# thunlp/ConvDR

Hardware: AMD Instinct MI355X
Metric: passages encoded/sec + query x passage IP-scored/sec, 768-d (higher is better)
Workload: dtype bf16

## Files before the change

convdr_amd/csrc/encoder_kernels.hpp:

```cpp
#pragma once
#include "../../include/convdr_hip.h"
#include "dropout.hpp"
#include "gemm_nt.hpp"

namespace convdr {

static __global__ void __launch_bounds__(256) k_seq_pack(const void* __restrict__ ids_v, int ids32,
                                                  const int64_t* __restrict__ mask, const int32_t* __restrict__ lens,
                                                  int B, int L, const int32_t* __restrict__ cu, int kind, int pad_idx,
                                                  int max_pos, int vocab, int32_t* __restrict__ tok_id,
                                                  int32_t* __restrict__ tok_pos, int32_t* __restrict__ status) {
  const int lane = threadIdx.x & 63;
  const int b = blockIdx.x * 4 + (threadIdx.x >> 6);
  if (b >= B) return;
  const int base = cu[b], end = cu[b + 1];
  const int64_t* ids = (const int64_t*)ids_v;
  const int32_t* ids_i = (const int32_t*)ids_v;
  const int len_b = lens[b];
  int kept = 0, nonpad = 0;
  int flags = 0;
  for (int l0 = 0; l0 < L; l0 += 64) {
    const int l = l0 + lane;
    const bool valid = l < L;
    int64_t id = valid ? (ids32 ? (int64_t)ids_i[(int64_t)b * L + l] : ids[(int64_t)b * L + l]) : (int64_t)pad_idx;
// ... 166 lines not shown
    const int e0 = 256 * j + 4 * lane;
    uint2 o;
    o.x = pack_bf16x2((x[j].x - mean) * rstd * gg[j].x + bb[j].x, (x[j].y - mean) * rstd * gg[j].y + bb[j].y);
    o.y = pack_bf16x2((x[j].z - mean) * rstd * gg[j].z + bb[j].z, (x[j].w - mean) * rstd * gg[j].w + bb[j].w);
    *(uint2*)(Xb + row * H + e0) = o;
  }
}

template <int J>
static __global__ void __launch_bounds__(256) k_slab_finish_ln(const float* __restrict__ slab, int nsplit, int64_t rows,
                                                               const float* __restrict__ bias, const bf16_t* __restrict__ R,
                                                               const float* __restrict__ g, const float* __restrict__ b, float eps,
                                                               bf16_t* __restrict__ Xb) {
  constexpr int H = 256 * J;
  const int lane = threadIdx.x & 63;
  const int64_t row = (int64_t)blockIdx.x * 4 + (threadIdx.x >> 6);
  if (row >= rows) return;
  float4 x[J], gg[J], bb[J], part[4][J];
  uint2 r[J];
#pragma unroll
  for (int j = 0; j < J; ++j) {
    const int e0 = 256 * j + 4 * lane;
    x[j] = *(const float4*)(bias + e0);
    gg[j] = *(const float4*)(g + e0);
    bb[j] = *(const float4*)(b + e0);
    r[j] = *(const uint2*)(R + row * H + e0);
#pragma unroll
    for (int s = 0; s < 4; ++s)
      part[s][j] = *(const float4*)(slab + ((int64_t)(s < nsplit ? s : 0) * rows + row) * H + e0);
  }
  float sum = 0.f;
#pragma unroll
  for (int j = 0; j < J; ++j) {
#pragma unroll
    for (int s = 0; s < 4; ++s)
      if (s < nsplit) { x[j].x += part[s][j].x; x[j].y += part[s][j].y; x[j].z += part[s][j].z; x[j].w += part[s][j].w; }
    x[j].x += __uint_as_float(r[j].x << 16); x[j].y += __uint_as_float(r[j].x & 0xffff0000u);
    x[j].z += __uint_as_float(r[j].y << 16); x[j].w += __uint_as_float(r[j].y & 0xffff0000u);
    sum += x[j].x + x[j].y + x[j].z + x[j].w;
  }
  const float mean = wave_sum(sum) / (float)H;
  float q = 0.f;
#pragma unroll
  for (int j = 0; j < J; ++j) {
    const float a = x[j].x - mean, c = x[j].y - mean, d = x[j].z - mean, e = x[j].w - mean;
    q += a * a + c * c + d * d + e * e;
  }
  const float rstd = rsqrtf(wave_sum(q) / (float)H + eps);
#pragma unroll
  for (int j = 0; j < J; ++j) {
    const int e0 = 256 * j + 4 * lane;
    uint2 o;
    o.x = pack_bf16x2((x[j].x - mean) * rstd * gg[j].x + bb[j].x, (x[j].y - mean) * rstd * gg[j].y + bb[j].y);
    o.y = pack_bf16x2((x[j].z - mean) * rstd * gg[j].z + bb[j].z, (x[j].w - mean) * rstd * gg[j].w + bb[j].w);
    *(uint2*)(Xb + row * H + e0) = o;
  }
}

inline int64_t g_ln_rows = 1;
static inline void launch_layernorm_bf16(const float* Y, int64_t rows, int H, const float* g, const float* b, float eps, bf16_t* Xb,
                                         hipStream_t st) {
  if (g_ln_rows && H == 768)
    hipLaunchKernelGGL(k_layernorm_rows<3>, dim3((unsigned)((rows + 3) / 4)), dim3(256), 0, st, Y, rows, g, b, eps, Xb);
  else
    hipLaunchKernelGGL(k_layernorm, dim3((unsigned)((rows + 3) / 4)), dim3(256), 0, st, Y, rows, H, g, b, eps, Xb, (float*)nullptr);
}

static __global__ void __launch_bounds__(256) k_gather_cls(const int32_t* __restrict__ cu, int B, int H,
                                                    const bf16_t* __restrict__ Xb, const float* __restrict__ Xf,
                                                    bf16_t* __restrict__ Ob, float* __restrict__ Of) {
  const int lane = threadIdx.x & 63;
  const int b = blockIdx.x * 4 + (threadIdx.x >> 6);
  if (b >= B) return;
  const int64_t row = cu[b];
  for (int e0 = 4 * lane; e0 < H; e0 += 256) {
    if (Ob) *(uint2*)(Ob + (int64_t)b * H + e0) = *(const uint2*)(Xb + row * H + e0);
    if (Of) *(float4*)(Of + (int64_t)b * H + e0) = *(const float4*)(Xf + row * H + e0);
  }
}

static __global__ void __launch_bounds__(256) k_masked_mean(const bf16_t* __restrict__ X, const int32_t* __restrict__ cu,
                                                     const int32_t* __restrict__ lens, int H, bf16_t* __restrict__ Ob,
                                                     float* __restrict__ Of) {
  const int b = blockIdx.x, c = 4 * threadIdx.x;
  if (c >= H) return;
  const int64_t base = cu[b];
  const int len = lens[b];
  float4 s = make_float4(0.f, 0.f, 0.f, 0.f);
  for (int t = 0; t < len; ++t) {
    const uint2 v = *(const uint2*)(X + (base + t) * H + c);
    s.x += __uint_as_float(v.x << 16); s.y += __uint_as_float(v.x & 0xffff0000u);
    s.z += __uint_as_float(v.y << 16); s.w += __uint_as_float(v.y & 0xffff0000u);
  }
  const float inv = 1.f / (float)len;
  s.x *= inv; s.y *= inv; s.z *= inv; s.w *= inv;
  if (Of) *(float4*)(Of + (int64_t)b * H + c) = s;
  if (Ob) {
    uint2 o;
    o.x = pack_bf16x2(s.x, s.y);
    o.y = pack_bf16x2(s.z, s.w);
    *(uint2*)(Ob + (int64_t)b * H + c) = o;
  }
}

enum { EPI_BF16 = 0, EPI_GELU_BF16 = 1, EPI_RESID_F32 = 2, EPI_QKV = 3, EPI_F32 = 4,
       EPI_GELU_SAVE = 5,
       EPI_SLAB_F32 = 7,
       EPI_GELU_BLK = 8,
       EPI_GELU_GP = 9,
       EPI_MUL_GP = 10 };
__host__ __device__ inline int64_t hm_blocked_offset(int64_t t, int f, int N) {
  return ((t >> 5) * (N >> 3) + (f >> 3)) * 256 + (t & 31) * 8 + (f & 7);
}

struct GemmArgs {
  const bf16_t* W;
  const bf16_t* X;
  int64_t rows;
  int N, K;
  int64_t ldw, ldx;
  int k_split_len;
  const float* bias;
  bf16_t* Cb;
  bf16_t* Cb2;
  float* Cf;
  const bf16_t* Gp;
  const bf16_t* R;
  const float* Rf;
  bf16_t *Qo, *Ko, *Vt;
  int third0;
  int qk_blocked;
  int H;
  int64_t ldt;
  int tilesN, tilesT;
  int tile_hint;
  int nt_out;
  int dbg_same_tile;
  int dbg_skip_epi;
  int dbg_prelanded;
  unsigned long long* trace;
  unsigned long long* clock_probe;
  DropSite drop;
};


__device__ __forceinline__ float gelu_tail(float x) {
  const float t = fminf(fabsf(x), 9.f);
  float p = fmaf(t, 0.0041585f, -0.04571999f);
  p = fmaf(p, t, -0.46495319f);
  p = fmaf(p, t, -1.14955714f);
  const float q = __builtin_amdgcn_exp2f(fmaf(p, t, -1.f));
  return fmaf(-t, q, fmaxf(x, 0.f));
}
__device__ __forceinline__ void gelu_tail2(float& x0, float& x1) {
  f32x2_t t, r;
  float a, b;
  const float nine = 9.f;
  asm("v_min_f32 %0, |%1|, %2" : "=v"(a) : "v"(x0), "s"(nine));
  asm("v_min_f32 %0, |%1|, %2" : "=v"(b) : "v"(x1), "s"(nine));
  t.x = a; t.y = b;
  asm("v_max_f32 %0, 0, %1" : "=v"(a) : "v"(x0));
  asm("v_max_f32 %0, 0, %1" : "=v"(b) : "v"(x1));
  r.x = a; r.y = b;
  const f32x2_t c3 = {0.0041585f, 0.0041585f}, c2 = {-0.04571999f, -0.04571999f}, c1 = {-0.46495319f, -0.46495319f},
                c0 = {-1.14955714f, -1.14955714f}, m1 = {-1.f, -1.f};
  f32x2_t p = __builtin_elementwise_fma(t, c3, c2);
  p = __builtin_elementwise_fma(p, t, c1);
  p = __builtin_elementwise_fma(p, t, c0);
  p = __builtin_elementwise_fma(p, t, m1);
  f32x2_t q;
  q.x = __builtin_amdgcn_exp2f(p.x);
  q.y = __builtin_amdgcn_exp2f(p.y);
  r = __builtin_elementwise_fma(-t, q, r);
  x0 = r.x; x1 = r.y;
}

__device__ __forceinline__ float gelu_grad(float x) {
  const float t = fminf(fabsf(x), 9.f);
  float p = fmaf(t, 0.0041585f, -0.04571999f);
  p = fmaf(p, t, -0.46495319f);
  p = fmaf(p, t, -1.14955714f);
  const float q = __builtin_amdgcn_exp2f(fmaf(p, t, -1.f));
  const float cdf = x >= 0.f ? 1.f - q : q;
  const float e = __builtin_amdgcn_exp2f(-0.7213475204444817f * x * x);
  return fmaf(x * 0.3989422804014327f, e, cdf);
}

__device__ __forceinline__ void gelu_tail2_gp(float& x0, float& x1, float& g0, float& g1) {
  f32x2_t t, r;
  float a, b;
  const float nine = 9.f;
  asm("v_min_f32 %0, |%1|, %2" : "=v"(a) : "v"(x0), "s"(nine));
  asm("v_min_f32 %0, |%1|, %2" : "=v"(b) : "v"(x1), "s"(nine));
  t.x = a; t.y = b;
  asm("v_max_f32 %0, 0, %1" : "=v"(a) : "v"(x0));
  asm("v_max_f32 %0, 0, %1" : "=v"(b) : "v"(x1));
  r.x = a; r.y = b;
  const f32x2_t c3 = {0.0041585f, 0.0041585f}, c2 = {-0.04571999f, -0.04571999f}, c1 = {-0.46495319f, -0.46495319f},
                c0 = {-1.14955714f, -1.14955714f}, m1 = {-1.f, -1.f};
  f32x2_t p = __builtin_elementwise_fma(t, c3, c2);
  p = __builtin_elementwise_fma(p, t, c1);
  p = __builtin_elementwise_fma(p, t, c0);
  p = __builtin_elementwise_fma(p, t, m1);
  f32x2_t q;
  q.x = __builtin_amdgcn_exp2f(p.x);
  q.y = __builtin_amdgcn_exp2f(p.y);
  const f32x2_t d4 = {-0.0117551f, -0.0117551f}, d3 = {0.09555683f, 0.09555683f}, d2 = {0.64461331f, 0.64461331f},
                d1 = {0.79644568f, 0.79644568f}, d0 = {-0.99992798f, -0.99992798f}, half = {0.5f, 0.5f};
  f32x2_t m = __builtin_elementwise_fma(t, d4, d3);
  m = __builtin_elementwise_fma(m, t, d2);
  m = __builtin_elementwise_fma(m, t, d1);
  m = __builtin_elementwise_fma(m, t, d0);
  const f32x2_t hr = __builtin_elementwise_fma(q, m, half);
  g0 = 0.5f + __builtin_copysignf(hr.x, x0);
  g1 = 0.5f + __builtin_copysignf(hr.y, x1);
  r = __builtin_elementwise_fma(-t, q, r);
  x0 = r.x; x1 = r.y;
}

template <class T>
struct CTile {
  static constexpr int PASSES = (T::TL * T::TR * 2) / T::STAGE_BYTES;
  static constexpr int NTP = T::NT / PASSES;
  static constexpr int ROWS = T::TL / PASSES;
  static_assert(PASSES >= 1 && PASSES * NTP == T::NT, "a pass is a whole number of MFMA column blocks");
  static constexpr int HALF = ROWS / 2, HALF_BYTES = HALF * T::TR * 2;
  struct Base { uint32_t lo, hi; };
  __device__ static __forceinline__ Base contiguous(const char* sC) {
    static_assert(2 * HALF_BYTES <= T::STAGE_BYTES, "a parked pass must fit the idle stage");
    return Base{lds_off(sC), lds_off(sC) + HALF_BYTES};
  }
  static constexpr int CW = T::MT * 4;
  static constexpr int RW = NTP * 32;
  static constexpr int W_BYTES = RW * CW * 16;
  static constexpr int W_STORES = RW * CW / 64;
  static_assert(W_BYTES * T::WAVES <= 2 * HALF_BYTES && (64 % CW) == 0, "wave-local park must fit the pass image");
  __device__ static __forceinline__ uint32_t wave_base(Base sC, int wave) {
    constexpr int PER_HALF = HALF_BYTES / W_BYTES;
    return (wave >= PER_HALF ? sC.hi + (wave - PER_HALF) * W_BYTES : sC.lo + wave * W_BYTES);
  }
  __device__ static __forceinline__ void put_w(uint32_t wb, const WavePos<T>& w, int mt, int ntl, int g, uint2 o) {
    const int row = ntl * 32 + w.li;
    lds_write_b64_hidden(wb + row * (CW * 16) + (((mt * 4 + g) ^ (row & (CW - 1))) << 4) + w.hi * 8, (u32x2_t){o.x, o.y});
  }
  template <int C0, int CN>
  __device__ static __forceinline__ void store_w_part(bool nt, uint32_t wb, int lane, bf16_t* dst, int64_t ld, int64_t row_limit,
                                                      int64_t col_limit) {
    constexpr int RPI = 64 / CN, N_ST = RW / RPI;
    static_assert(64 % CN == 0 && N_ST % 4 == 0, "store_w_part geometry");
    const int r0 = lane / CN, c = C0 + (lane - r0 * CN);
    const int64_t nv = col_limit - c * 8;
#pragma unroll
    for (int i0 = 0; i0 < N_ST; i0 += 4) {
      u32x4_t v[4];
      auto at = [&](int i) {
        const int row = i * RPI + r0;
        return wb + row * (CW * 16) + ((c ^ (row & (CW - 1))) << 4);
      };
      lds_read4_b128_hidden(at(i0), at(i0 + 1), at(i0 + 2), at(i0 + 3), v[0], v[1], v[2], v[3]);
#pragma unroll
      for (int j = 0; j < 4; ++j) {
        const int row = (i0 + j) * RPI + r0;
        bf16_t* pr = dst + (int64_t)row * ld + c * 8;
        if (row < row_limit && nv > 0) {
          if (nv >= 8) {
            if (nt) store16<true>(pr, v[j]);
            else store16<false>(pr, v[j]);
          }
          else *(uint2*)pr = make_uint2(v[j].x, v[j].y);
        }
      }
    }
  }
  __device__ static __forceinline__ void store_w(bool nt, uint32_t wb, int lane, bf16_t* dst, int64_t ld, int64_t row_limit,
                                                 int64_t col_limit) {
    constexpr int RPI = 64 / CW;
    const int r0 = lane / CW, c = lane - r0 * CW;
    const int64_t nv = col_limit - c * 8;
    static_assert(W_STORES % 4 == 0, "lds_read4_b128_hidden reads four chunks");
#pragma unroll
    for (int i0 = 0; i0 < W_STORES; i0 += 4) {
      u32x4_t v[4];
      auto at = [&](int i) {
        const int row = i * RPI + r0;
        return wb + row * (CW * 16) + ((c ^ (row & (CW - 1))) << 4);
      };
      lds_read4_b128_hidden(at(i0), at(i0 + 1), at(i0 + 2), at(i0 + 3), v[0], v[1], v[2], v[3]);
#pragma unroll
      for (int j = 0; j < 4; ++j) {
        const int row = (i0 + j) * RPI + r0;
        bf16_t* pr = dst + (int64_t)row * ld + c * 8;
        if (row < row_limit && nv > 0) {
          if (nv >= 8) {
            if (nt) store16<true>(pr, v[j]);
            else store16<false>(pr, v[j]);
          }
          else *(uint2*)pr = make_uint2(v[j].x, v[j].y);
        }
      }
    }
  }
};

template <int EPI, class T>
static __global__ void __launch_bounds__(T::THREADS, 2) k_gemm(const GemmArgs a) {
  extern __shared__ __attribute__((aligned(16))) char smem[];
  using CT = CTile<T>;
  const WavePos<T> w;
  const int64_t ldw = a.ldw ? a.ldw : a.K, ldx = a.ldx ? a.ldx : a.K;
  int kbeg = 0, klen = a.K;
  if constexpr (EPI == EPI_SLAB_F32) {
    if (a.k_split_len) { kbeg = blockIdx.y * a.k_split_len; klen = a.k_split_len; }
  }
  const uint32_t ntiles = (uint32_t)a.tilesN * a.tilesT;
  const uint32_t xcd = blockIdx.x & 7u, q8 = ntiles >> 3, r8 = ntiles & 7u;
  const uint32_t chunk_base = xcd < r8 ? xcd * (q8 + 1) : r8 * (q8 + 1) + (xcd - r8) * q8;
  const uint32_t chunk_len = q8 + (xcd < r8 ? 1u : 0u);
  const uint32_t stride = (gridDim.x + 7u) >> 3;
  uint32_t idx = blockIdx.x >> 3;
  if (idx >= chunk_len) return;
  if (a.clock_probe && blockIdx.x == 0 && blockIdx.y == 0 && threadIdx.x == 0) {
    a.clock_probe[0] = __builtin_amdgcn_s_memtime();
    a.clock_probe[1] = __builtin_amdgcn_s_memrealtime();
  }

  struct Coord { int64_t t0; int n0; int swap; };
  auto decode = [&](uint32_t i) {
    const uint32_t logical = chunk_base + i;
    int tt = logical / a.tilesN, tn = logical - tt * a.tilesN;
    if (a.dbg_same_tile) { tt = 0; tn = 0; }
    Coord c;
    c.t0 = (int64_t)tt * T::TL;
    c.n0 = tn * T::TR;
    c.swap = false;
    if constexpr (EPI == EPI_QKV) c.swap = c.n0 + a.third0 * a.H >= 2 * a.H;
    return c;
  };
  auto tile_src = [&](const Coord& c) {
    return c.swap ? TileSrc<T>(a.X, ldx, a.rows, a.W, ldw, a.N, c.t0, c.n0, w)
                  : TileSrc<T>(a.W + kbeg, ldw, a.N, a.X + kbeg, ldx, a.rows, c.n0, c.t0, w);
  };

  constexpr bool R3 = T::WAVES == 8;
  R3Slots st{0, 0};
  auto sbias_of = [&](R3Slots s) { return (float*)(smem + (s.rs == 2 ? 0 : s.rs + 1) * T::R_BYTES); };
  auto tile_src_all = [&](const Coord& cc) {
    return cc.swap ? TileSrcAll<T>(a.X, ldx, a.rows, a.W, ldw, a.N, cc.t0, cc.n0, w)
                   : TileSrcAll<T>(a.W + kbeg, ldw, a.N, a.X + kbeg, ldx, a.rows, cc.n0, cc.t0, w);
  };
  float* sbias = R3 ? sbias_of(st) : (float*)(smem + T::SMEM_BYTES);
  int trace_tile = 0;
#ifdef CONVDR_ENABLE_TRACE
#define CONVDR_TRACE(ph)                                                                                       \
  if (a.trace && threadIdx.x == 0 && trace_tile < 64)                                                          \
    a.trace[((size_t)blockIdx.x * 64 + trace_tile) * 16 + (ph)] = __builtin_amdgcn_s_memtime();
#else
#define CONVDR_TRACE(ph)
#endif
  auto bias_slice = [&](const Coord& cc) {
    const int f = cc.n0 + (int)threadIdx.x;
    return (!cc.swap && a.bias && threadIdx.x < T::TR && f < a.N) ? a.bias[f] : 0.f;
  };
  Coord c = decode(idx);
  int buf = 0;
  bool landed = false;
  if (threadIdx.x < T::TR) sbias[threadIdx.x] = bias_slice(c);
  TileSrc<T> src = tile_src(c);
  TileSrcAll<T> src3 = tile_src_all(c);
  if constexpr (R3) gemm_r3_prologue<T>(src3, a.K, smem, w, st, false);
  else gemm_issue_stage<T>(src, 0, smem + buf * T::STAGE_BYTES, w);
  __syncthreads();
  for (;;) {
    const uint32_t next = idx + stride;
    const bool has_next = next < chunk_len;
    const Coord cn = has_next ? decode(next) : c;
    GemmAcc<T> acc;
    float bias_lane[T::NT];
    if (c.swap) {
      acc.zero();
#pragma unroll
      for (int nt = 0; nt < T::NT; ++nt) {
        const int f = c.n0 + w.l_index(nt);
        bias_lane[nt] = a.bias[f < a.N ? f : a.N - 1];
      }
    } else {
#pragma unroll
      for (int nt = 0; nt < T::NT; ++nt) bias_lane[nt] = 0.f;
#pragma unroll
      for (int mt = 0; mt < T::MT; ++mt) {
        u32x4_t bq[4];
        const uint32_t sb = lds_off(sbias);
        lds_read4_b128_hidden(sb + w.r_base(mt, 0) * 4, sb + w.r_base(mt, 1) * 4, sb + w.r_base(mt, 2) * 4,
                              sb + w.r_base(mt, 3) * 4, bq[0], bq[1], bq[2], bq[3]);
#pragma unroll
        for (int g = 0; g < 4; ++g)
#pragma unroll
          for (int nt = 0; nt < T::NT; ++nt) {
            acc.c[mt][nt][4 * g + 0] = __uint_as_float(bq[g].x); acc.c[mt][nt][4 * g + 1] = __uint_as_float(bq[g].y);
            acc.c[mt][nt][4 * g + 2] = __uint_as_float(bq[g].z); acc.c[mt][nt][4 * g + 3] = __uint_as_float(bq[g].w);
          }
      }
    }
    float bias_next = has_next ? bias_slice(cn) : 0.f;
    constexpr bool RES_PRE = EPI == EPI_RESID_F32 && T::WAVES == 4;
    uint2 res_pre[RES_PRE ? T::NT : 1][T::MT][4];
    if constexpr (RES_PRE) {
      if (a.Rf == nullptr) {
#pragma unroll
        for (int nt = 0; nt < T::NT; ++nt) {
          const int64_t t = c.t0 + w.l_index(nt);
          const int64_t tc = t < a.rows ? t : a.rows - 1;
#pragma unroll
          for (int mt = 0; mt < T::MT; ++mt)
#pragma unroll
            for (int g = 0; g < 4; ++g) {
              int f = c.n0 + w.r_base(mt, g);
              f = f < a.N ? f : a.N - 4;
              res_pre[nt][mt][g] = *(const uint2*)(a.R + tc * a.N + f);
            }
        }
      }
    }
    CONVDR_TRACE(0)
    int idle;
    if constexpr (R3) {
      st = gemm_nt_mainloop_r3<T>(src3, c.swap ? a.K : klen, smem, acc, w, st, true, true, landed || a.dbg_prelanded,
                                  (a.trace && trace_tile == 8) ? a.trace + ((size_t)blockIdx.x * 64 + 56) * 16 : nullptr);
      idle = 0;
      sbias = sbias_of(st);
    } else {
    idle = gemm_nt_mainloop<T>(src, c.swap ? a.K : klen, smem, acc, w, buf, true, landed,
                               (a.trace && trace_tile == 8) ? a.trace + ((size_t)blockIdx.x * 64 + 56) * 16 : nullptr);
    }
    landed = false;
    constexpr bool GP_PRE = EPI == EPI_MUL_GP;
    u32x4_t gp_pre[GP_PRE ? T::NT : 1][GP_PRE ? T::MT : 1][2];
    if constexpr (GP_PRE) {
      int tid_p = threadIdx.x;
      asm volatile("" : "+v"(tid_p));
      const WavePos<T> wp(tid_p);
      const int64_t rows32p = (a.rows + 31) & ~(int64_t)31;
#pragma unroll
      for (int nt = 0; nt < T::NT; ++nt) {
        const int64_t tb = c.t0 + (wp.wl * T::NT + nt) * 32;
        const int64_t tbc = tb < rows32p ? tb : 0;
#pragma unroll
        for (int mt = 0; mt < T::MT; ++mt) {
          const int f0 = c.n0 + wp.wr * T::MT * 32 + mt * 32;
          const int f0c = f0 < a.N ? f0 : 0;
          const bf16_t* blk = a.Gp + ((tbc >> 5) * (a.N >> 3) + (f0c >> 3)) * 256 + wp.li * 8;
#pragma unroll
          for (int j = 0; j < 2; ++j)
            gp_pre[nt][mt][j] = __builtin_nontemporal_load((const u32x4_t*)(blk + (int64_t)(2 * j + wp.hi) * 256));
        }
      }
    }
    asm volatile("" : "+v"(bias_next));
    if constexpr (RES_PRE) {
#pragma unroll
      for (int nt = 0; nt < T::NT; ++nt)
#pragma unroll
        for (int mt = 0; mt < T::MT; ++mt)
#pragma unroll
          for (int g = 0; g < 4; ++g) asm volatile("" : "+v"(res_pre[nt][mt][g].x), "+v"(res_pre[nt][mt][g].y));
    }
#pragma unroll
    for (int i = 0; i < T::NT; ++i) asm volatile("" : "+v"(bias_lane[i]));
    if (threadIdx.x < T::TR) sbias[threadIdx.x] = bias_next;
    CONVDR_TRACE(1)
    if (has_next) {
      if constexpr (R3) {
        src3 = tile_src_all(cn);
        gemm_r3_prologue<T>(src3, a.K, smem, w, st, false);
      } else {
        src = tile_src(cn);
        gemm_issue_stage<T>(src, 0, smem + idle * T::STAGE_BYTES, w);
      }
    }
    typename CT::Base sC;
    if constexpr (R3) {
      static_assert(T::R_BYTES >= CT::HALF_BYTES && 3 * T::R_BYTES + 2 * T::L_BYTES + (T::L_BYTES >= CT::HALF_BYTES ? 0 : CT::HALF_BYTES) <= 160 * 1024,
                    "parked pass: one dead R slot + one dead L slot (or the spare LDS behind the slots)");
      sC = typename CT::Base{lds_off(smem + (st.rs == 0 ? 2 : st.rs - 1) * T::R_BYTES),
                             T::L_BYTES >= CT::HALF_BYTES ? lds_off(smem + 3 * T::R_BYTES + (st.ls ^ 1) * T::L_BYTES)
                                                          : lds_off(smem + 3 * T::R_BYTES + 2 * T::L_BYTES)};
    } else {
      sC = CT::contiguous(smem + (idle ^ 1) * T::STAGE_BYTES);
    }
    int tid_e = threadIdx.x;
    asm volatile("" : "+v"(tid_e));
    const WavePos<T> we(tid_e);
    const int64_t t0 = c.t0;
    const int n0 = c.n0;

    if (a.dbg_skip_epi == 1) {
      float s = 0.f;
#pragma unroll
      for (int mt = 0; mt < T::MT; ++mt)
#pragma unroll
        for (int nt = 0; nt < T::NT; ++nt)
#pragma unroll
          for (int r = 0; r < 16; ++r) s += acc.c[mt][nt][r];
      if (s == 12345.678f) a.Cb[0] = f32_to_bf16(s);
    } else if (c.swap) {
      lds_barrier();
#pragma unroll
      for (int pass = 0; pass < CT::PASSES; ++pass) {
        const uint32_t wb = CT::wave_base(sC, we.wave);
#pragma unroll
        for (int ntl = 0; ntl < CT::NTP; ++ntl) {
          const int nt = pass * CT::NTP + ntl;
          const float bv = bias_lane[nt];
#pragma unroll
          for (int mt = 0; mt < T::MT; ++mt)
#pragma unroll
            for (int g = 0; g < 4; ++g) {
              const f32x16& v = acc.c[mt][nt];
              uint2 o;
              o.x = pack_bf16x2(v[4 * g + 0] + bv, v[4 * g + 1] + bv);
              o.y = pack_bf16x2(v[4 * g + 2] + bv, v[4 * g + 3] + bv);
              CT::put_w(wb, we, mt, ntl, g, o);
            }
        }
        if (pass == CT::PASSES - 1 && has_next) {
          lds_dma_wait_all();
          landed = true;
        }
        const int row0 = (we.wl * T::NT + pass * CT::NTP) * 32, col0 = we.wr * T::MT * 32;
        CT::store_w(a.nt_out != 0, wb, we.lane, a.Vt + (int64_t)(n0 + (a.third0 - 2) * a.H + row0) * a.ldt + t0 + col0, a.ldt,
                    a.N - n0 - row0, a.rows - t0 - col0);
      }
    } else if (EPI == EPI_GELU_BLK || (EPI == EPI_QKV && a.qk_blocked)) {
      lds_barrier();
      CONVDR_TRACE(2)
      const int64_t rows32 = (a.rows + 31) & ~(int64_t)31;
      bf16_t* dstm = a.Cb;
      int oct_w = a.N >> 3, f0 = n0;
      if constexpr (EPI == EPI_QKV) {
        const int na = n0 + a.third0 * a.H;
        dstm = na < a.H ? a.Qo : a.Ko;
        f0 = na < a.H ? na : na - a.H;
        oct_w = a.H >> 3;
      }
#pragma unroll
      for (int nt = 0; nt < T::NT; ++nt) {
        const int64_t tb = t0 + (we.wl * T::NT + nt) * 32;
        if (nt == T::NT - 1 && has_next) {
          lds_dma_wait_all();
          landed = true;
        }
        bf16_t* blk = dstm + ((tb >> 5) * oct_w + ((f0 + we.wr * T::MT * 32) >> 3)) * 256 + we.li * 8;
#pragma unroll
        for (int mt = 0; mt < T::MT; ++mt)
#pragma unroll
          for (int j = 0; j < 2; ++j) {
            uint2 o[2];
#pragma unroll
            for (int e = 0; e < 2; ++e) {
              const int g = 2 * j + e;
              const f32x16& v = acc.c[mt][nt];
              float y0 = v[4 * g + 0], y1 = v[4 * g + 1], y2 = v[4 * g + 2], y3 = v[4 * g + 3];
              if constexpr (EPI == EPI_GELU_BLK) { gelu_tail2(y0, y1); gelu_tail2(y2, y3); }
              o[e].x = pack_bf16x2(y0, y1);
              o[e].y = pack_bf16x2(y2, y3);
            }
            const auto sx = __builtin_amdgcn_permlane32_swap(o[0].x, o[1].x, false, false);
            const auto sy = __builtin_amdgcn_permlane32_swap(o[0].y, o[1].y, false, false);
            u32x4_t q;
            q.x = sx[0]; q.y = sy[0]; q.z = sx[1]; q.w = sy[1];
            if (tb < rows32 && n0 + we.wr * T::MT * 32 + mt * 32 < a.N)
              store16<NT_GEMM_BLK>(blk + (int64_t)(mt * 4 + 2 * j + we.hi) * 256, q);
          }
      }
      CONVDR_TRACE(6)
    } else {
      lds_barrier();
      CONVDR_TRACE(2)
      const bool full_n = n0 + T::TR <= a.N;
      constexpr bool BF16_OUT = EPI == EPI_BF16 || EPI == EPI_GELU_BF16 || EPI == EPI_QKV || EPI == EPI_GELU_SAVE ||
                                EPI == EPI_GELU_GP || EPI == EPI_MUL_GP;
      constexpr bool GP = EPI == EPI_GELU_GP || EPI == EPI_MUL_GP;
      const int64_t rows32 = (a.rows + 31) & ~(int64_t)31;
      constexpr int NOUT = EPI == EPI_GELU_SAVE ? 2 : 1;
#pragma unroll
      for (int out = 0; out < NOUT; ++out)
#pragma unroll
        for (int pass = 0; pass < CT::PASSES; ++pass) {
          const uint32_t wb = CT::wave_base(sC, we.wave);
          constexpr bool HALVES = BF16_OUT && T::MT >= 4 && CT::NTP == 1;
          bf16_t* wdst = nullptr;
          int64_t wld = 0, wrows = 0, wcols = 0;
          if constexpr (HALVES) {
            bf16_t* dst;
            int64_t cols;
            if constexpr (EPI == EPI_QKV) {
              const int na = n0 + a.third0 * a.H;
              dst = na < a.H ? a.Qo + t0 * a.H + na : a.Ko + t0 * a.H + (na - a.H);
              wld = a.H; cols = T::TR;
            } else {
              dst = (out ? a.Cb2 : a.Cb) + t0 * a.N + n0;
              wld = a.N; cols = a.N - n0;
            }
            const int row0 = (we.wl * T::NT + pass * CT::NTP) * 32, col0 = we.wr * T::MT * 32;
            wdst = dst + (int64_t)row0 * wld + col0; wrows = a.rows - t0 - row0; wcols = cols - col0;
          }
#pragma unroll
          for (int ntl = 0; ntl < CT::NTP; ++ntl) {
            const int nt = pass * CT::NTP + ntl;
            const int64_t t = t0 + we.l_index(nt);
            const bool t_ok = t < a.rows;
            const int64_t tc = t_ok ? t : a.rows - 1;
            uint2 res[T::MT][4];
            u32x4_t gpq[GP ? T::MT : 1][2];
            bf16_t* gp_blk = nullptr;
            bool gp_ok = false;
            if constexpr (GP) {
              const int64_t tb = t0 + (we.wl * T::NT + nt) * 32;
              bf16_t* img = EPI == EPI_GELU_GP ? a.Cb2 : const_cast<bf16_t*>(a.Gp);
              gp_blk = img + ((tb >> 5) * (a.N >> 3) + ((n0 + we.wr * T::MT * 32) >> 3)) * 256 + we.li * 8;
              gp_ok = tb < rows32;
              if constexpr (EPI == EPI_MUL_GP) {
#pragma unroll
                for (int mt = 0; mt < T::MT; ++mt)
#pragma unroll
                  for (int j = 0; j < 2; ++j) gpq[mt][j] = gp_pre[nt][mt][j];
              }
            }
            if constexpr (EPI == EPI_RESID_F32) {
              if (a.Rf == nullptr) {
#pragma unroll
                for (int mt = 0; mt < T::MT; ++mt)
#pragma unroll
                  for (int g = 0; g < 4; ++g) {
                    if constexpr (RES_PRE) {
                      res[mt][g] = res_pre[nt][mt][g];
                    } else {
                      int f = n0 + we.r_base(mt, g);
                      f = (full_n || f < a.N) ? f : a.N - 4;
                      res[mt][g] = *(const uint2*)(a.R + tc * a.N + f);
                    }
                  }
              }
            }
            uint2 gpq_o0 = make_uint2(0u, 0u), gpq_o1 = make_uint2(0u, 0u);
#pragma unroll
            for (int mt = 0; mt < T::MT; ++mt)
#pragma unroll
              for (int g = 0; g < 4; ++g) {
                const int fl = we.r_base(mt, g);
                const int f = n0 + fl;
                const f32x16& v = acc.c[mt][nt];
                float y0 = v[4 * g + 0], y1 = v[4 * g + 1], y2 = v[4 * g + 2], y3 = v[4 * g + 3];
                if constexpr (EPI == EPI_GELU_BF16 || EPI == EPI_GELU_SAVE) {
                  if (out == 0) {
                    gelu_tail2(y0, y1); gelu_tail2(y2, y3);
                  }
                }
                if constexpr (EPI == EPI_GELU_GP) {
                  float d0, d1, d2, d3;
                  gelu_tail2_gp(y0, y1, d0, d1); gelu_tail2_gp(y2, y3, d2, d3);
                  uint2& dq = (g & 1) ? gpq_o1 : gpq_o0;
                  dq.x = pack_bf16x2(d0, d1);
                  dq.y = pack_bf16x2(d2, d3);
                  if (g & 1) {
                    const auto sx = __builtin_amdgcn_permlane32_swap(gpq_o0.x, gpq_o1.x, false, false);
                    const auto sy = __builtin_amdgcn_permlane32_swap(gpq_o0.y, gpq_o1.y, false, false);
                    u32x4_t q4;
                    q4.x = sx[0]; q4.y = sy[0]; q4.z = sx[1]; q4.w = sy[1];
                    if (gp_ok && (full_n || f < a.N))
                      store16<true>(gp_blk + (int64_t)(mt * 4 + (g & 2) + we.hi) * 256, q4);
                  }
                }
                if constexpr (EPI == EPI_MUL_GP) {
                  if (!(g & 1)) {
                    const u32x4_t q4 = gpq[mt][g >> 1];
                    const auto sx = __builtin_amdgcn_permlane32_swap(q4.x, q4.z, false, false);
                    const auto sy = __builtin_amdgcn_permlane32_swap(q4.y, q4.w, false, false);
                    gpq_o0 = make_uint2(sx[0], sy[0]);
                    gpq_o1 = make_uint2(sx[1], sy[1]);
                  }
                  const uint2 dq = (g & 1) ? gpq_o1 : gpq_o0;
                  y0 *= __uint_as_float(dq.x << 16); y1 *= __uint_as_float(dq.x & 0xffff0000u);
                  y2 *= __uint_as_float(dq.y << 16); y3 *= __uint_as_float(dq.y & 0xffff0000u);
                }
                if constexpr (EPI == EPI_RESID_F32) {
                  if (a.drop.thresh) {
                    float m0, m1, m2, m3;
                    drop_hidden4(a.drop, t, f, a.N, m0, m1, m2, m3);
                    y0 *= m0; y1 *= m1; y2 *= m2; y3 *= m3;
                  }
                  if (a.Rf) {
                    const int fc = (full_n || f < a.N) ? f : a.N - 4;
                    const float4 r = *(const float4*)(a.Rf + tc * a.N + fc);
                    y0 += r.x; y1 += r.y; y2 += r.z; y3 += r.w;
                  } else {
                    const uint2 r = res[mt][g];
                    y0 += __uint_as_float(r.x << 16); y1 += __uint_as_float(r.x & 0xffff0000u);
                    y2 += __uint_as_float(r.y << 16); y3 += __uint_as_float(r.y & 0xffff0000u);
                  }
                }
                if constexpr (BF16_OUT) {
                  uint2 o;
                  o.x = pack_bf16x2(y0, y1);
                  o.y = pack_bf16x2(y2, y3);
                  CT::put_w(wb, we, mt, ntl, g, o);
                  if constexpr (HALVES) {
                    if (mt == T::MT / 2 - 1 && g == 3) {
                      if (out == NOUT - 1 && pass == CT::PASSES - 1 && has_next) { lds_dma_wait_all(); landed = true; }
                      CT::template store_w_part<0, CT::CW / 2>(a.nt_out != 0, wb, we.lane, wdst, wld, wrows, wcols);
                    }
                  }
                } else if (t_ok && (full_n || f < a.N)) {
                  if constexpr (EPI == EPI_SLAB_F32) {
                    *(float4*)(a.Cf + ((int64_t)blockIdx.y * a.rows + t) * a.N + f) = make_float4(y0, y1, y2, y3);
                  } else {
                    *(float4*)(a.Cf + t * a.N + f) = make_float4(y0, y1, y2, y3);
                  }
                }
              }
          }
          CONVDR_TRACE(3 + 4 * pass)
          if constexpr (BF16_OUT) {
            CONVDR_TRACE(4 + 4 * pass)
            if (out == NOUT - 1 && pass == CT::PASSES - 1 && has_next) {
              lds_dma_wait_all();
              landed = true;
            }
            CONVDR_TRACE(5 + 4 * pass)
            if (a.dbg_skip_epi != 3) {
              bf16_t* dst;
              int64_t ldo, cols;
              if constexpr (EPI == EPI_QKV) {
                const int na = n0 + a.third0 * a.H;
                dst = na < a.H ? a.Qo + t0 * a.H + na : a.Ko + t0 * a.H + (na - a.H);
// ... 268 lines not shown
```

convdr_amd/csrc/gemm_nt.hpp:

```cpp
#pragma once
#include "common.hpp"

namespace convdr {

constexpr int GEMM_BK = 64;

typedef const __attribute__((address_space(1))) void* gptr_t;
typedef __attribute__((address_space(3))) void* lptr_t;

__device__ __forceinline__ void glds16(const void* g, void* lds_wave_base) {
  __builtin_amdgcn_global_load_lds((gptr_t)g, (lptr_t)lds_wave_base, 16, 0, 0);
}
template <bool NT, class V>
__device__ __forceinline__ void store16(void* p, const V& v) {
  static_assert(sizeof(V) == 16, "16-byte store");
  typedef uint32_t raw4_t __attribute__((ext_vector_type(4)));
  if constexpr (NT) __builtin_nontemporal_store(__builtin_bit_cast(raw4_t, v), (raw4_t*)p);
  else *(V*)p = v;
}
constexpr bool NT_GEMM_BLK = true;
constexpr bool NT_CTILE = true;
constexpr bool NT_ATT = true;
constexpr bool NT_LN = true;
template <int AUX>
__device__ __forceinline__ void glds16_aux(const void* g, void* lds_wave_base) {
  __builtin_amdgcn_global_load_lds((gptr_t)g, (lptr_t)lds_wave_base, 16, 0, AUX);
}

__device__ __forceinline__ void lds_dma_wait_all() { asm volatile("s_waitcnt vmcnt(0)" ::: "memory"); }

__device__ __forceinline__ void lds_barrier() { asm volatile("s_waitcnt lgkmcnt(0)\n\ts_barrier" ::: "memory"); }

typedef uint32_t u32x4_t __attribute__((ext_vector_type(4)));
typedef uint32_t u32x2_t __attribute__((ext_vector_type(2)));
__device__ __forceinline__ uint32_t lds_off(const void* p) {
  return (uint32_t)(uintptr_t)(__attribute__((address_space(3))) const char*)p;
}
__device__ __forceinline__ void lds_write_b64_hidden(uint32_t addr, u32x2_t v) {
  asm volatile("ds_write_b64 %0, %1" ::"v"(addr), "v"(v) : "memory");
}
__device__ __forceinline__ void lds_read4_b128_hidden(uint32_t a0, uint32_t a1, uint32_t a2, uint32_t a3, u32x4_t& v0,
                                                      u32x4_t& v1, u32x4_t& v2, u32x4_t& v3) {
  asm volatile(
      "ds_read_b128 %0, %4\n\tds_read_b128 %1, %5\n\tds_read_b128 %2, %6\n\tds_read_b128 %3, %7\n\t"
      "s_waitcnt lgkmcnt(0)"
      : "=&v"(v0), "=&v"(v1), "=&v"(v2), "=&v"(v3)
      : "v"(a0), "v"(a1), "v"(a2), "v"(a3)
      : "memory");
}

typedef _Float16 f16x8 __attribute__((ext_vector_type(8)));
template <bool F16>
__device__ __forceinline__ f32x16 mfma_32x32x16(const bf16x8& a, const bf16x8& b, const f32x16& c) {
  if constexpr (F16)
    return __builtin_amdgcn_mfma_f32_32x32x16_f16(__builtin_bit_cast(f16x8, a), __builtin_bit_cast(f16x8, b), c, 0, 0, 0);
  else
    return __builtin_amdgcn_mfma_f32_32x32x16_bf16(a, b, c, 0, 0, 0);
}

template <int WR_, int WL_, int MT_, int NT_>
struct TileCfg {
  static constexpr int WR = WR_, WL = WL_, MT = MT_, NT = NT_;
  static constexpr int TR = WR * MT * 32, TL = WL * NT * 32;
  static constexpr int WAVES = WR * WL, THREADS = WAVES * 64;
  static constexpr int DMA_WAVES = WAVES == 8 ? 4 : WAVES;
  static constexpr int DMA_FIRST = WAVES - DMA_WAVES;
  static constexpr int R_BYTES = TR * 128, L_BYTES = TL * 128;
  static constexpr int STAGE_BYTES = R_BYTES + L_BYTES;
  static constexpr int SMEM_BYTES = 2 * STAGE_BYTES;
  static constexpr int MIN_WAVES_PER_SIMD = THREADS >= 512 ? 2 : 2;
};
using Tile128 = TileCfg<2, 2, 2, 2>;
using Tile256 = TileCfg<2, 4, 4, 2>;
using TileTall = TileCfg<2, 4, 4, 1>;
using TileWide = TileCfg<4, 2, 2, 2>;

template <class T>
struct GemmAcc {
  f32x16 c[T::MT][T::NT];
  __device__ __forceinline__ void zero() {
#pragma unroll
    for (int i = 0; i < T::MT; ++i)
#pragma unroll
      for (int j = 0; j < T::NT; ++j)
#pragma unroll
        for (int r = 0; r < 16; ++r) c[i][j][r] = 0.f;
  }
};

template <class T>
struct WavePos {
  int lane, wave, wr, wl, hi, li;
  __device__ __forceinline__ WavePos() : WavePos((int)threadIdx.x) {}
  __device__ __forceinline__ explicit WavePos(int tid) {
    lane = tid & 63;
    wave = __builtin_amdgcn_readfirstlane(tid >> 6);
    wr = wave / T::WL;
    wl = wave - wr * T::WL;
    hi = lane >> 5;
    li = lane & 31;
  }
  __device__ __forceinline__ int r_base(int mt, int g) const { return (wr * T::MT + mt) * 32 + 8 * g + 4 * hi; }
  __device__ __forceinline__ int r_index(int mt, int r) const { return (wr * T::MT + mt) * 32 + (r & 3) + 8 * (r >> 2) + 4 * hi; }
  __device__ __forceinline__ int l_index(int nt) const { return (wl * T::NT + nt) * 32 + li; }
};

typedef int32_t i32x4_t __attribute__((ext_vector_type(4)));

struct StageSrc {
  __amdgpu_buffer_rsrc_t rsrc;
  uint32_t voff;
  uint32_t round_pitch;
};

template <int WAVES, int FIRST>
__device__ __forceinline__ StageSrc gemm_stage_src(const bf16_t* __restrict__ G, int64_t ld, int64_t row0, int64_t nrows,
                                                    int wave, int lane) {
  wave = wave >= FIRST ? wave - FIRST : 0;
  StageSrc s;
  int64_t bytes = (nrows - row0) * ld * 2;
  bytes = bytes < 0 ? 0 : (bytes > 0xffffffffll ? 0xffffffffll : bytes);
  const uint64_t base = (uint64_t)(G + row0 * ld);
  const uint32_t lo = __builtin_amdgcn_readfirstlane((uint32_t)base);
  const uint32_t hi = __builtin_amdgcn_readfirstlane((uint32_t)(base >> 32));
  const uint32_t nb = __builtin_amdgcn_readfirstlane((uint32_t)bytes);
  s.rsrc = __builtin_amdgcn_make_buffer_rsrc((void*)(((uint64_t)hi << 32) | lo), 0, nb, 0x00020000);
  const int row = wave * 8 + (lane >> 3);
  const int gch = (lane & 7) ^ ((row >> 1) & 7);
  s.voff = (uint32_t)(row * ld * 2) + gch * 16;
  s.round_pitch = __builtin_amdgcn_readfirstlane((uint32_t)(8 * WAVES * ld * 2));
  return s;
}

template <int ROWS, int WAVES, int FIRST, int AUX = 0>
__device__ __forceinline__ void gemm_stage(const StageSrc& s, int kt, char* lds_tile, int wave) {
  if (FIRST > 0 && wave < FIRST) return;
  wave -= FIRST;
  constexpr int ROUNDS = ROWS / (8 * WAVES);
  static_assert(ROUNDS * 8 * WAVES == ROWS, "tile rows must be a multiple of 8 * waves");
#pragma unroll
  for (int i = 0; i < ROUNDS; ++i)
    __builtin_amdgcn_raw_ptr_buffer_load_lds(s.rsrc, (lptr_t)(lds_tile + (i * WAVES + wave) * 8 * 128), 16, s.voff,
                                             i * s.round_pitch + kt * (GEMM_BK * 2), 0, AUX);
}

template <class T>
struct TileSrc {
  StageSrc R, L;
  __device__ __forceinline__ TileSrc(const bf16_t* __restrict__ Rp, int64_t ldr, int64_t nR, const bf16_t* __restrict__ Lp,
                                     int64_t ldl, int64_t nL, int64_t r0, int64_t l0, const WavePos<T>& w)
      : R(gemm_stage_src<T::DMA_WAVES, T::DMA_FIRST>(Rp, ldr, r0, nR, w.wave, w.lane)),
        L(gemm_stage_src<T::DMA_WAVES, T::DMA_FIRST>(Lp, ldl, l0, nL, w.wave, w.lane)) {}
};

template <class T>
__device__ __forceinline__ void gemm_issue_stage(const TileSrc<T>& src, int kt, char* stage, const WavePos<T>& w) {
  gemm_stage<T::TR, T::DMA_WAVES, T::DMA_FIRST>(src.R, kt, stage, w.wave);
  gemm_stage<T::TL, T::DMA_WAVES, T::DMA_FIRST>(src.L, kt, stage + T::R_BYTES, w.wave);
}

template <class T, bool F16 = false>
__device__ __forceinline__ int gemm_nt_mainloop(const TileSrc<T>& src, int K, char* smem, GemmAcc<T>& acc,
                                                const WavePos<T>& w, int first_buf = 0, bool stage0_in_flight = false,
                                                bool stage0_landed = false, unsigned long long* step_trace = nullptr) {
  const int nk = K / GEMM_BK;
  const int sw = (w.lane >> 1) & 7;
  const int offR = (w.wr * T::MT * 32 + w.li) * 128;
  const int offL = T::R_BYTES + (w.wl * T::NT * 32 + w.li) * 128;

  if (!stage0_in_flight) gemm_issue_stage<T>(src, 0, smem + first_buf * T::STAGE_BYTES, w);

  for (int kt = 0; kt < nk; ++kt) {
    const int buf = (kt + first_buf) & 1;
#ifdef CONVDR_ENABLE_TRACE
#define CONVDR_STEP_TRACE(i) \
  if (step_trace && kt == 6 + (i) / 5 && w.lane == 0) step_trace[w.wave * 8 + (i)] = __builtin_amdgcn_s_memtime();
#else
#define CONVDR_STEP_TRACE(i)
#endif
    CONVDR_STEP_TRACE(5)
    CONVDR_STEP_TRACE(0)
    if (kt > 0 || !stage0_landed) lds_dma_wait_all();
    CONVDR_STEP_TRACE(1)
    lds_barrier();
    CONVDR_STEP_TRACE(2)
    if (kt + 1 < nk) gemm_issue_stage<T>(src, kt + 1, smem + (buf ^ 1) * T::STAGE_BYTES, w);
    CONVDR_STEP_TRACE(3)
    const char* tR = smem + buf * T::STAGE_BYTES + offR;
    const char* tL = smem + buf * T::STAGE_BYTES + offL;
    bf16x8 fa[2][T::MT], fb[2][T::NT];
    auto load_frags = [&](int s, int set) {
      const int ch = ((2 * s + w.hi) ^ sw) * 16;
#pragma unroll
      for (int j = 0; j < T::NT; ++j) fb[set][j] = *(const bf16x8*)(tL + j * 32 * 128 + ch);
#pragma unroll
      for (int i = 0; i < T::MT; ++i) fa[set][i] = *(const bf16x8*)(tR + i * 32 * 128 + ch);
    };
    load_frags(0, 0);
#pragma unroll
    for (int s = 0; s < 4; ++s) {
      if (s + 1 < 4) load_frags(s + 1, (s + 1) & 1);
#pragma unroll
      for (int i = 0; i < T::MT; ++i)
#pragma unroll
        for (int j = 0; j < T::NT; ++j)
          acc.c[i][j] = mfma_32x32x16<F16>(fa[s & 1][i], fb[s & 1][j], acc.c[i][j]);
      if (s + 1 < 4) {
#pragma unroll
        for (int r = 0; r < T::MT + T::NT && r < T::MT * T::NT; ++r) {
          __builtin_amdgcn_sched_group_barrier(0x008, 1, 0);
          __builtin_amdgcn_sched_group_barrier(0x100, 1, 0);
        }
        __builtin_amdgcn_sched_group_barrier(0x100, T::MT + T::NT, 0);
        __builtin_amdgcn_sched_group_barrier(0x008, T::MT * T::NT, 0);
      }
      __builtin_amdgcn_sched_barrier(0);
    }
    CONVDR_STEP_TRACE(4)
  }
  return (nk + first_buf) & 1;
}

template <class T>
struct R3Issue {
  static constexpr bool ROLES = T::WAVES == 8;
  static constexpr int RW = ROLES ? T::WAVES / 2 : T::WAVES;
  static constexpr int LW = ROLES ? T::WAVES / 2 : T::WAVES;
  static constexpr int LFIRST = ROLES ? T::WAVES / 2 : 0;
  static constexpr int R_DPW = T::TR / (8 * RW);
  static __device__ __forceinline__ bool issues_r(int wave) { return !ROLES || wave < RW; }
  template <int AUX = 0>
  static __device__ __forceinline__ void r(const StageSrc& s, int kt, char* dst, int wave) {
    if (issues_r(wave)) gemm_stage<T::TR, RW, 0, AUX>(s, kt, dst, wave);
  }
  static __device__ __forceinline__ void l(const StageSrc& s, int kt, char* dst, int wave) {
    gemm_stage<T::TL, LW, LFIRST>(s, kt, dst, wave);
  }
};
template <class T>
struct TileSrcAll {
  StageSrc R, L;
  __device__ __forceinline__ TileSrcAll(const bf16_t* __restrict__ Rp, int64_t ldr, int64_t nR, const bf16_t* __restrict__ Lp,
                                        int64_t ldl, int64_t nL, int64_t r0, int64_t l0, const WavePos<T>& w)
      : R(gemm_stage_src<R3Issue<T>::RW, 0>(Rp, ldr, r0, nR, w.wave, w.lane)),
        L(gemm_stage_src<R3Issue<T>::LW, R3Issue<T>::LFIRST>(Lp, ldl, l0, nL, w.wave, w.lane)) {}
};
struct R3Slots { int rs, ls; };
template <class T, int R_AUX = 0>
__device__ __forceinline__ void gemm_r3_prologue(const TileSrcAll<T>& src, int K, char* smem, const WavePos<T>& w, R3Slots s,
                                                 bool with_r1 = true) {
  char* sR = smem;
  char* sL = smem + 3 * T::R_BYTES;
  R3Issue<T>::template r<R_AUX>(src.R, 0, sR + s.rs * T::R_BYTES, w.wave);
  R3Issue<T>::l(src.L, 0, sL + s.ls * T::L_BYTES, w.wave);
  if (with_r1 && K > GEMM_BK) R3Issue<T>::template r<R_AUX>(src.R, 1, sR + (s.rs == 2 ? 0 : s.rs + 1) * T::R_BYTES, w.wave);
}
template <class T, bool F16 = false, int R_AUX = 0>
__device__ __forceinline__ R3Slots gemm_nt_mainloop_r3(const TileSrcAll<T>& src, int K, char* smem, GemmAcc<T>& acc,
                                                       const WavePos<T>& w, R3Slots st = R3Slots{0, 0},
                                                       bool prologue_in_flight = false, bool r1_deferred = false,
                                                       bool stage0_landed = false, unsigned long long* step_trace = nullptr) {
  constexpr int R_DPW = R3Issue<T>::R_DPW;
  const bool r_wave = R3Issue<T>::issues_r(w.wave);
  const int nk = K / GEMM_BK;
  const int sw = (w.lane >> 1) & 7;
  const int offR = (w.wr * T::MT * 32 + w.li) * 128;
  const int offL = (w.wl * T::NT * 32 + w.li) * 128;
  char* sR = smem;
  char* sL = smem + 3 * T::R_BYTES;
  if (!prologue_in_flight) gemm_r3_prologue<T, R_AUX>(src, K, smem, w, st, !r1_deferred);
  int rs = st.rs, ls = st.ls;
#ifdef CONVDR_ENABLE_TRACE
#define CONVDR_R3_STEP(i) \
  if (step_trace && kt == 6 + (i) / 6 && w.lane == 0) step_trace[w.wave * 8 + (i)] = __builtin_amdgcn_s_memtime();
#else
#define CONVDR_R3_STEP(i)
#endif
  for (int kt = 0; kt < nk; ++kt) {
    CONVDR_R3_STEP(6)
    CONVDR_R3_STEP(0)
    if (kt == 0 && (r1_deferred || stage0_landed)) {
      if (!stage0_landed) lds_dma_wait_all();
    } else if (kt + 1 < nk && r_wave) asm volatile("s_waitcnt vmcnt(%0)" ::"n"(R_DPW) : "memory");
    else lds_dma_wait_all();
    CONVDR_R3_STEP(1)
    lds_barrier();
    CONVDR_R3_STEP(2)
    const char* tR = sR + rs * T::R_BYTES + offR;
    const char* tL = sL + ls * T::L_BYTES + offL;
    bf16x8 fa[2][T::MT], fb[2][T::NT];
    auto load_frags = [&](int s, int set) {
      const int ch = ((2 * s + w.hi) ^ sw) * 16;
#pragma unroll
      for (int j = 0; j < T::NT; ++j) fb[set][j] = *(const bf16x8*)(tL + j * 32 * 128 + ch);
#pragma unroll
      for (int i = 0; i < T::MT; ++i) fa[set][i] = *(const bf16x8*)(tR + i * 32 * 128 + ch);
    };
    load_frags(0, 0);
    const bool issue_l = kt + 1 < nk, issue_r = kt + 2 < nk;
    char* l_dst = sL + (ls ^ 1) * T::L_BYTES;
    const int rnext = rs == 0 ? 2 : rs - 1;
    char* r_dst = sR + rnext * T::R_BYTES;
    __builtin_amdgcn_sched_barrier(0);
    if (r1_deferred && kt == 0 && issue_l) R3Issue<T>::template r<R_AUX>(src.R, 1, sR + (rs == 2 ? 0 : rs + 1) * T::R_BYTES, w.wave);
    if (issue_l) R3Issue<T>::l(src.L, kt + 1, l_dst, w.wave);
    CONVDR_R3_STEP(3)
#pragma unroll
    for (int s = 0; s < 4; ++s) {
      if (s + 1 < 4) load_frags(s + 1, (s + 1) & 1);
#pragma unroll
      for (int i = 0; i < T::MT; ++i)
#pragma unroll
        for (int j = 0; j < T::NT; ++j)
          acc.c[i][j] = mfma_32x32x16<F16>(fa[s & 1][i], fb[s & 1][j], acc.c[i][j]);
      if (s + 1 < 4) {
#pragma unroll
        for (int r = 0; r < T::MT + T::NT && r < T::MT * T::NT; ++r) {
          __builtin_amdgcn_sched_group_barrier(0x008, 1, 0);
          __builtin_amdgcn_sched_group_barrier(0x100, 1, 0);
        }
        __builtin_amdgcn_sched_group_barrier(0x100, T::MT + T::NT, 0);
        __builtin_amdgcn_sched_group_barrier(0x008, T::MT * T::NT, 0);
      }
      __builtin_amdgcn_sched_barrier(0);
    }
    CONVDR_R3_STEP(4)
    if (issue_r) R3Issue<T>::template r<R_AUX>(src.R, kt + 2, r_dst, w.wave);
    CONVDR_R3_STEP(5)
    rs = rs == 2 ? 0 : rs + 1;
    ls ^= 1;
  }
  return R3Slots{rs, ls};
}

template <class T>
__device__ __forceinline__ int gemm_nt_mainloop(const bf16_t* __restrict__ R, int64_t ldr, int64_t nR,
                                                const bf16_t* __restrict__ L, int64_t ldl, int64_t nL, int K,
                                                int64_t r0, int64_t l0, char* smem, GemmAcc<T>& acc,
                                                const WavePos<T>& w, int k_begin = 0) {
  const TileSrc<T> src(R + k_begin, ldr, nR, L + k_begin, ldl, nL, r0, l0, w);
  return gemm_nt_mainloop<T>(src, K, smem, acc, w);
}

}
```

Measured before the change: 45280.

## Use 16x16x32 MFMA mainloop for GELU and QKV GEMM epilogues

Adds an alternative GEMM mainloop that issues 16x16x32 MFMA instructions in place of 32x32x16, with a matching LDS fragment read pattern. The accumulator is remapped into the existing 32x32 layout using permlane16 swaps, so the epilogues stay unchanged. The new path is selected at compile time for the GELU and QKV epilogues in both the double-buffer and the triple-buffer mainloops. It aims for better MFMA/LDS scheduling or issue rate on those shapes, at the cost of more LDS reads per FLOP and extra register shuffling around the loop.

Result: no change. 45920 (median of 6 runs) (+1.4%).

```diff
diff --git a/convdr_amd/csrc/encoder_kernels.hpp b/convdr_amd/csrc/encoder_kernels.hpp
--- a/convdr_amd/csrc/encoder_kernels.hpp
+++ b/convdr_amd/csrc/encoder_kernels.hpp
@@ -492,6 +492,9 @@
   }
 };
 
+constexpr MfmaShape gemm_epi_shape(int epi) {
+  return (epi == EPI_GELU_BLK || epi == EPI_GELU_BF16 || epi == EPI_QKV) ? MfmaShape::M16N16K32 : MfmaShape::M32N32K16;
+}
 template <int EPI, class T>
 static __global__ void __launch_bounds__(T::THREADS, 2) k_gemm(const GemmArgs a) {
   extern __shared__ __attribute__((aligned(16))) char smem[];
@@ -614,12 +617,12 @@
     CONVDR_TRACE(0)
     int idle;
     if constexpr (R3) {
-      st = gemm_nt_mainloop_r3<T>(src3, c.swap ? a.K : klen, smem, acc, w, st, true, true, landed || a.dbg_prelanded,
+      st = gemm_nt_mainloop_r3<T, false, 0, gemm_epi_shape(EPI)>(src3, c.swap ? a.K : klen, smem, acc, w, st, true, true, landed || a.dbg_prelanded,
                                   (a.trace && trace_tile == 8) ? a.trace + ((size_t)blockIdx.x * 64 + 56) * 16 : nullptr);
       idle = 0;
       sbias = sbias_of(st);
     } else {
-    idle = gemm_nt_mainloop<T>(src, c.swap ? a.K : klen, smem, acc, w, buf, true, landed,
+    idle = gemm_nt_mainloop<T, false, gemm_epi_shape(EPI)>(src, c.swap ? a.K : klen, smem, acc, w, buf, true, landed,
                                (a.trace && trace_tile == 8) ? a.trace + ((size_t)blockIdx.x * 64 + 56) * 16 : nullptr);
     }
     landed = false;
diff --git a/convdr_amd/csrc/gemm_nt.hpp b/convdr_amd/csrc/gemm_nt.hpp
--- a/convdr_amd/csrc/gemm_nt.hpp
+++ b/convdr_amd/csrc/gemm_nt.hpp
@@ -56,6 +56,16 @@
     return __builtin_amdgcn_mfma_f32_32x32x16_f16(__builtin_bit_cast(f16x8, a), __builtin_bit_cast(f16x8, b), c, 0, 0, 0);
   else
     return __builtin_amdgcn_mfma_f32_32x32x16_bf16(a, b, c, 0, 0, 0);
+}
+
+enum class MfmaShape { M32N32K16, M16N16K32 };
+
+template <bool F16>
+__device__ __forceinline__ f32x4 mfma_16x16x32(const bf16x8& a, const bf16x8& b, const f32x4& c) {
+  if constexpr (F16)
+    return __builtin_amdgcn_mfma_f32_16x16x32_f16(__builtin_bit_cast(f16x8, a), __builtin_bit_cast(f16x8, b), c, 0, 0, 0);
+  else
+    return __builtin_amdgcn_mfma_f32_16x16x32_bf16(a, b, c, 0, 0, 0);
 }
 
 template <int WR_, int WL_, int MT_, int NT_>
@@ -103,6 +113,88 @@
   __device__ __forceinline__ int r_base(int mt, int g) const { return (wr * T::MT + mt) * 32 + 8 * g + 4 * hi; }
   __device__ __forceinline__ int r_index(int mt, int r) const { return (wr * T::MT + mt) * 32 + (r & 3) + 8 * (r >> 2) + 4 * hi; }
   __device__ __forceinline__ int l_index(int nt) const { return (wl * T::NT + nt) * 32 + li; }
+};
+
+template <class T>
+struct Acc16 {
+  static constexpr int FR = 2 * T::MT, FL = 2 * T::NT;
+  f32x4 q[FR][FL];
+  __device__ __forceinline__ static void swap_pairs(GemmAcc<T>& acc) {
+#pragma unroll
+    for (int mt = 0; mt < T::MT; ++mt)
+#pragma unroll
+      for (int nt = 0; nt < T::NT; ++nt)
+#pragma unroll
+        for (int m = 0; m < 2; ++m)
+#pragma unroll
+          for (int e = 0; e < 4; ++e) {
+            const auto r = __builtin_amdgcn_permlane16_swap(__float_as_uint(acc.c[mt][nt][8 * m + e]),
+                                                            __float_as_uint(acc.c[mt][nt][8 * m + 4 + e]), false, false);
+            acc.c[mt][nt][8 * m + e] = __uint_as_float(r[0]);
+            acc.c[mt][nt][8 * m + 4 + e] = __uint_as_float(r[1]);
+          }
+  }
+  __device__ __forceinline__ void from(GemmAcc<T>& acc) {
+    swap_pairs(acc);
+#pragma unroll
+    for (int i = 0; i < FR; ++i)
+#pragma unroll
+      for (int jj = 0; jj < FL; ++jj)
+#pragma unroll
+        for (int e = 0; e < 4; ++e) q[i][jj][e] = acc.c[i >> 1][jj >> 1][4 * (2 * (i & 1) + (jj & 1)) + e];
+  }
+  __device__ __forceinline__ void to(GemmAcc<T>& acc) const {
+#pragma unroll
+    for (int i = 0; i < FR; ++i)
+#pragma unroll
+      for (int jj = 0; jj < FL; ++jj)
+#pragma unroll
+        for (int e = 0; e < 4; ++e) acc.c[i >> 1][jj >> 1][4 * (2 * (i & 1) + (jj & 1)) + e] = q[i][jj][e];
+    swap_pairs(acc);
+  }
+};
+template <class T, bool F16>
+struct KStep16 {
+  static constexpr int FR = Acc16<T>::FR, FL = Acc16<T>::FL;
+  static_assert(FL <= FR, "one L fragment of the next sub-step is read per R fragment");
+  int offR, offL, swR, swL, q;
+  __device__ __forceinline__ explicit KStep16(const WavePos<T>& w) {
+    const int l15 = w.lane & 15;
+    const int ar = (l15 & 3) | ((l15 & 4) << 1) | ((l15 & 8) >> 1);
+    q = w.lane >> 4;
+    offR = (w.wr * T::MT * 32 + ar) * 128;
+    offL = (w.wl * T::NT * 32 + l15) * 128;
+    swR = (ar >> 1) & 7;
+    swL = (l15 >> 1) & 7;
+  }
+  template <class F>
+  __device__ __forceinline__ void run(const char* tR, const char* tL, Acc16<T>& acc, F&& after_first_reads) const {
+    bf16x8 fb[2][FL], fa[3];
+    auto rd_a = [&](int n) { return *(const bf16x8*)(tR + (n % FR) * 16 * 128 + ((4 * (n / FR) + q) ^ swR) * 16); };
+    auto rd_b = [&](int s, int j) { return *(const bf16x8*)(tL + j * 16 * 128 + ((4 * s + q) ^ swL) * 16); };
+#pragma unroll
+    for (int j = 0; j < FL; ++j) fb[0][j] = rd_b(0, j);
+    fa[0] = rd_a(0);
+    fa[1] = rd_a(1);
+    __builtin_amdgcn_sched_barrier(0);
+    after_first_reads();
+#pragma unroll
+    for (int n = 0; n < 2 * FR; ++n) {
+      const int s = n / FR, i = n % FR;
+      const int reads = (n + 2 < 2 * FR ? 1 : 0) + (s == 0 && i < FL ? 1 : 0);
+      if (n + 2 < 2 * FR) fa[(n + 2) % 3] = rd_a(n + 2);
+      if (s == 0 && i < FL) fb[1][i] = rd_b(1, i);
+#pragma unroll
+      for (int j = 0; j < FL; ++j) acc.q[i][j] = mfma_16x16x32<F16>(fa[n % 3], fb[s][j], acc.q[i][j]);
+#pragma unroll
+      for (int r = 0; r < reads; ++r) {
+        __builtin_amdgcn_sched_group_barrier(0x008, 1, 0);
+        __builtin_amdgcn_sched_group_barrier(0x100, 1, 0);
+      }
+      __builtin_amdgcn_sched_group_barrier(0x008, FL, 0);
+      __builtin_amdgcn_sched_barrier(0);
+    }
+  }
 };
 
 typedef int32_t i32x4_t __attribute__((ext_vector_type(4)));
@@ -159,7 +251,7 @@
   gemm_stage<T::TL, T::DMA_WAVES, T::DMA_FIRST>(src.L, kt, stage + T::R_BYTES, w.wave);
 }
 
-template <class T, bool F16 = false>
+template <class T, bool F16 = false, MfmaShape SHAPE = MfmaShape::M32N32K16>
 __device__ __forceinline__ int gemm_nt_mainloop(const TileSrc<T>& src, int K, char* smem, GemmAcc<T>& acc,
                                                 const WavePos<T>& w, int first_buf = 0, bool stage0_in_flight = false,
                                                 bool stage0_landed = false, unsigned long long* step_trace = nullptr) {
@@ -170,6 +262,20 @@
 
   if (!stage0_in_flight) gemm_issue_stage<T>(src, 0, smem + first_buf * T::STAGE_BYTES, w);
 
+  if constexpr (SHAPE == MfmaShape::M16N16K32) {
+    const KStep16<T, F16> ks(w);
+    Acc16<T> a16;
+    a16.from(acc);
+    for (int kt = 0; kt < nk; ++kt) {
+      const int buf = (kt + first_buf) & 1;
+      if (kt > 0 || !stage0_landed) lds_dma_wait_all();
+      lds_barrier();
+      if (kt + 1 < nk) gemm_issue_stage<T>(src, kt + 1, smem + (buf ^ 1) * T::STAGE_BYTES, w);
+      ks.run(smem + buf * T::STAGE_BYTES + ks.offR, smem + buf * T::STAGE_BYTES + T::R_BYTES + ks.offL, a16, [] {});
+    }
+    a16.to(acc);
+    return (nk + first_buf) & 1;
+  }
   for (int kt = 0; kt < nk; ++kt) {
     const int buf = (kt + first_buf) & 1;
 #ifdef CONVDR_ENABLE_TRACE
@@ -255,7 +361,7 @@
   R3Issue<T>::l(src.L, 0, sL + s.ls * T::L_BYTES, w.wave);
   if (with_r1 && K > GEMM_BK) R3Issue<T>::template r<R_AUX>(src.R, 1, sR + (s.rs == 2 ? 0 : s.rs + 1) * T::R_BYTES, w.wave);
 }
-template <class T, bool F16 = false, int R_AUX = 0>
+template <class T, bool F16 = false, int R_AUX = 0, MfmaShape SHAPE = MfmaShape::M32N32K16>
 __device__ __forceinline__ R3Slots gemm_nt_mainloop_r3(const TileSrcAll<T>& src, int K, char* smem, GemmAcc<T>& acc,
                                                        const WavePos<T>& w, R3Slots st = R3Slots{0, 0},
                                                        bool prologue_in_flight = false, bool r1_deferred = false,
@@ -270,6 +376,10 @@
   char* sL = smem + 3 * T::R_BYTES;
   if (!prologue_in_flight) gemm_r3_prologue<T, R_AUX>(src, K, smem, w, st, !r1_deferred);
   int rs = st.rs, ls = st.ls;
+  constexpr bool S16 = SHAPE == MfmaShape::M16N16K32;
+  const KStep16<T, F16> ks16(w);
+  Acc16<T> a16;
+  if constexpr (S16) a16.from(acc);
 #ifdef CONVDR_ENABLE_TRACE
 #define CONVDR_R3_STEP(i) \
   if (step_trace && kt == 6 + (i) / 6 && w.lane == 0) step_trace[w.wave * 8 + (i)] = __builtin_amdgcn_s_memtime();
@@ -286,6 +396,22 @@
     CONVDR_R3_STEP(1)
     lds_barrier();
     CONVDR_R3_STEP(2)
+    if constexpr (SHAPE == MfmaShape::M16N16K32) {
+      const bool issue_l = kt + 1 < nk, issue_r = kt + 2 < nk;
+      char* l_dst = sL + (ls ^ 1) * T::L_BYTES;
+      char* r_dst = sR + (rs == 0 ? 2 : rs - 1) * T::R_BYTES;
+      ks16.run(sR + rs * T::R_BYTES + ks16.offR, sL + ls * T::L_BYTES + ks16.offL, a16, [&] {
+        if (r1_deferred && kt == 0 && issue_l) R3Issue<T>::template r<R_AUX>(src.R, 1, sR + (rs == 2 ? 0 : rs + 1) * T::R_BYTES, w.wave);
+        if (issue_l) R3Issue<T>::l(src.L, kt + 1, l_dst, w.wave);
+        CONVDR_R3_STEP(3)
+      });
+      CONVDR_R3_STEP(4)
+      if (issue_r) R3Issue<T>::template r<R_AUX>(src.R, kt + 2, r_dst, w.wave);
+      CONVDR_R3_STEP(5)
+      rs = rs == 2 ? 0 : rs + 1;
+      ls ^= 1;
+      continue;
+    }
     const char* tR = sR + rs * T::R_BYTES + offR;
     const char* tL = sL + ls * T::L_BYTES + offL;
     bf16x8 fa[2][T::MT], fb[2][T::NT];
@@ -330,6 +456,7 @@
     rs = rs == 2 ? 0 : rs + 1;
     ls ^= 1;
   }
+  if constexpr (S16) a16.to(acc);
   return R3Slots{rs, ls};
 }
 
```
